# theovincent/iS-DQN

Measured on AMD Instinct MI355X. Metric: gradient-steps/sec (batch=256, K=9, 84x84x4), higher is better.
Workload: dtype bf16x3 (split-bf16 MFMA operands hi+lo, fp32 accumulate)

## Files before the change

is-dqn_amd/csrc/common.h:

```cpp
#pragma once
#include <hip/hip_runtime.h>
#include <stdint.h>
#include <stdio.h>
#include <stdlib.h>

#include "../../include/isdqn_hip.h"

namespace isdqn {

void set_last_error(const char* fmt, ...);

#define ISDQN_HIP_CHECK(expr)                                                                         \
    do {                                                                                              \
        hipError_t _e = (expr);                                                                       \
        if (_e != hipSuccess) {                                                                       \
            ::isdqn::set_last_error("%s failed: %s (%s:%d)", #expr, hipGetErrorString(_e), __FILE__, \
                                    __LINE__);                                                        \
            return ISDQN_ERR_HIP;                                                                     \
        }                                                                                             \
    } while (0)

#define ISDQN_REQUIRE(cond, code, msg)                                         \
    do {                                                                       \
        if (!(cond)) {                                                         \
            ::isdqn::set_last_error("%s (%s:%d)", msg, __FILE__, __LINE__);    \
            return code;                                                       \
        }                                                                      \
    } while (0)

struct FastDiv {
    uint32_t d, m, sh;
    __host__ __device__ FastDiv() : d(1), m(0), sh(0) {}
    __host__ __device__ explicit FastDiv(uint32_t div) : d(div), m(0), sh(0) {
        if (div > 1) {
            uint32_t lg = 0;
            while ((1u << lg) < div) ++lg;
            uint32_t p = 31 + lg;
            m = (uint32_t)(((1ull << p) + div - 1) / div);
            sh = p - 32;
        }
    }
    __host__ __device__ __forceinline__ uint32_t div(uint32_t n) const {
#if defined(__HIP_DEVICE_COMPILE__)
        const uint32_t q = __umulhi(n, m) >> sh;
        return d == 1 ? n : q;
#else
        return d == 1 ? n : (uint32_t)((((uint64_t)n * m) >> 32) >> sh);
#endif
    }
    __host__ __device__ __forceinline__ void divmod(uint32_t n, uint32_t& q, uint32_t& r) const {
        q = div(n);
        r = n - q * d;
    }
};

#if defined(ISDQN_DEV)
#define ISDQN_DEV_ENV(name) (getenv(name) != nullptr)
#else
#define ISDQN_DEV_ENV(name) (false)
#endif

#if defined(ISDQN_DEV)
#define ISDQN_REPORT_OCCUPANCY(kernel, threads, lds_bytes, grid)                                                              \
    do {                                                                                                                      \
        static bool reported_ = false;                                                                                        \
        if (!reported_ && getenv("ISDQN_DEBUG_OCCUPANCY")) {                                                                  \
            reported_ = true;                                                                                                 \
            int nb_ = 0;                                                                                                      \
            if (hipOccupancyMaxActiveBlocksPerMultiprocessor(&nb_, reinterpret_cast<const void*>(kernel), (threads),          \
                                                             (lds_bytes)) == hipSuccess)                                      \
                fprintf(stderr, "[isdqn] %s: grid %d x %d threads, %d B LDS -> %d workgroups per CU\n", __PRETTY_FUNCTION__,  \
                        (int)(grid), (int)(threads), (int)(lds_bytes), nb_);                                                  \
        }                                                                                                                     \
    } while (0)
#else
#define ISDQN_REPORT_OCCUPANCY(kernel, threads, lds_bytes, grid) do {} while (0)
#endif

constexpr int ISDQN_MAX_DEVICES = 16;
static inline int current_device_slot() {
    int d = 0;
    if (hipGetDevice(&d) != hipSuccess || d < 0 || d >= ISDQN_MAX_DEVICES) d = 0;
    return d;
}
struct LdsConfigured {
    int bytes[ISDQN_MAX_DEVICES] = {0};
};
template <class F>
static inline int ensure_dynamic_lds(F kernel, int lds_bytes, LdsConfigured& state) {
    if (lds_bytes <= 65536) return ISDQN_OK;
    const int d = current_device_slot();
    if (lds_bytes > state.bytes[d]) {
        ISDQN_HIP_CHECK(hipFuncSetAttribute(reinterpret_cast<const void*>(kernel), hipFuncAttributeMaxDynamicSharedMemorySize, lds_bytes));
        state.bytes[d] = lds_bytes;
    }
    return ISDQN_OK;
}

static inline int ceil_div(int a, int b) { return (a + b - 1) / b; }
static inline int round_up(int a, int b) { return ceil_div(a, b) * b; }

}

#if defined(ISDQN_EMPTY)
#define ISDQN_EMPTY_KERNEL_RETURN return;
#else
#define ISDQN_EMPTY_KERNEL_RETURN
#endif
```

is-dqn_amd/csrc/conv_img.h:

```cpp
#pragma once
#include "net_problems.h"

namespace isdqn {

__device__ __forceinline__ int column_slot(int c16) { return c16 < 4 ? 8 + c16 : (c16 < 12 ? c16 - 4 : c16); }
struct PixelOrder {
    int strips;
    int n_full;
    int full_w;
    FastDiv d_h8, d_rem, d_w;
    PixelOrder() : strips(0), n_full(0), full_w(0) {}
    PixelOrder(int H, int W, bool use_strips) : strips(use_strips ? 1 : 0), n_full(H * 8 * (W / 8)), full_w(8 * (W / 8)) {
        d_h8 = FastDiv((uint32_t)(H * 8));
        d_rem = FastDiv((uint32_t)(W % 8 ? W % 8 : 1));
        d_w = FastDiv((uint32_t)W);
    }
    __device__ __forceinline__ void map(int n, int& y, int& x) const {
        uint32_t a, b;
        if (!strips) {
            d_w.divmod((uint32_t)n, a, b);
            y = (int)a; x = (int)b;
        } else if (n < n_full) {
            d_h8.divmod((uint32_t)n, a, b);
            y = (int)(b >> 3); x = (int)(a * 8 + (b & 7));
// ... 680 lines not shown
            int pixoff[2], arow[2];
#pragma unroll
            for (int h = 0; h < 2; ++h) {
                int kp = ks * GEMM_BK + tr_row(8 * grp + 4 * h + q);
                arow[h] = kp * p.PA + 4 * pq;
                kp = kp < g.npix ? kp : g.npix - 1;
                uint32_t oy, ox;
                g.d_wout.divmod((uint32_t)kp, oy, ox);
                pixoff[h] = U8 ? ((int)oy * g.stride * p.Wp + (int)ox * g.stride)
                               : ((int)oy * g.stride * p.Wp + (int)ox * g.stride) * p.PPin;
            }
            bf16x8 fa_hi[MT], fa_lo[MT];
#pragma unroll
            for (int mt = 0; mt < MT; ++mt) {
                fa_hi[mt] = tr_frag(dzi + arow[0] + mt * 16, dzi + arow[1] + mt * 16);
                if constexpr (PASSES >= 2)
                    fa_lo[mt] = tr_frag(dzi + p.dz_plane + arow[0] + mt * 16, dzi + p.dz_plane + arow[1] + mt * 16);
            }
#pragma unroll
            for (int t = 0; t < NTW; ++t) {
                const __bf16* b0 = img + pixoff[0] + col_off[t];
                const __bf16* b1 = img + pixoff[1] + col_off[t];
                bf16x8 fb_hi = tr_frag(b0, b1), fb_lo;
                if constexpr (PASSES >= 3) fb_lo = tr_frag(b0 + p.in_plane, b1 + p.in_plane);
#pragma unroll
                for (int mt = 0; mt < MT; ++mt) {
                    if constexpr (PASSES >= 3)
                        mfma_acc(acc[mt][t], fa_hi[mt], fb_lo);
                    if constexpr (PASSES >= 2)
                        mfma_acc(acc[mt][t], fa_lo[mt], fb_hi);
                    mfma_acc(acc[mt][t], fa_hi[mt], fb_hi);
                }
            }
        }
    };
    bool staged = false;
    if constexpr (!U8) {
        if (p.prefetch) {
            staged = true;
            ImagePrefetch<WgradPrefetch<WV>::DZ> ra;
            ImagePrefetch<WgradPrefetch<WV>::IN> rb;
            auto request = [&](int j) {
                request_image_s8<NTHR>(ra, p.dz + (int64_t)j * g.npix * g.cout_p, 1, g.npix, g.cout_p, 0, 0, 1, p.npix_pad, p.PA, tid,
                                       p.d_dzchunk, p.d_npixpad);
                request_image_s8<NTHR>(rb, p.in + (int64_t)j * g.hin * g.win * g.cin_p, g.hin, g.win, g.cin_p, -g.pad, -g.pad, p.R, p.Wp,
                                       p.PPin, tid, p.d_chunk, p.d_Wp);
            };
            request(j0);
            for (int j = j0; j < j1; ++j) {
                __syncthreads();
                commit_image_s8<A_PLANES>(dzi, p.dz_plane, ra);
                commit_image_s8<B_PLANES>(img, p.in_plane, rb);
                __syncthreads();
                if (j == j0) { WG_STAMP(1); } else if (j == j0 + 1) { WG_STAMP(3); }
                if (j + 1 < j1) request(j + 1);
                k_steps();
                if (j == j0) { WG_STAMP(2); } else if (j == j0 + 1) { WG_STAMP(4); }
            }
        }
    }
    if (!staged)
    for (int j = j0; j < j1; ++j) {
        __syncthreads();
        bool dz_done = false;
        if constexpr (U8) {
            if (p.prefetch) {
                ImagePrefetch<WgradPrefetch<WV>::DZ_U8> ra;
                request_image_s8<NTHR>(ra, p.dz + (int64_t)j * g.npix * g.cout_p, 1, g.npix, g.cout_p, 0, 0, 1, p.npix_pad, p.PA, tid,
                                       p.d_dzchunk, p.d_npixpad);
                fill_input_image<U8, PASSES, NTHR>(img, p.in_plane, g, p.fs, p.in, j, -g.pad, p.R, p.Wp, p.PPin, tid, p.d_chunk, p.d_Wp, p.d_R);
                commit_image_s8<A_PLANES>(dzi, p.dz_plane, ra);
                dz_done = true;
            }
        }
        if (!dz_done) {
            fill_image_s8<NTHR, A_PLANES, 8>(dzi, p.dz_plane, p.dz + (int64_t)j * g.npix * g.cout_p, 1, g.npix, g.cout_p, 0, 0, 1, p.npix_pad,
                                             p.PA, tid, p.d_dzchunk, p.d_npixpad);
            fill_input_image<U8, PASSES, NTHR>(img, p.in_plane, g, p.fs, p.in, j, -g.pad, p.R, p.Wp, p.PPin, tid, p.d_chunk, p.d_Wp, p.d_R);
        }
        __syncthreads();
        if (j == j0) { WG_STAMP(1); } else if (j == j0 + 1) { WG_STAMP(3); }
        k_steps();
        if (j == j0) { WG_STAMP(2); } else if (j == j0 + 1) { WG_STAMP(4); }
    }

    float* slab = p.slabs + (int64_t)ig * g.cout_p * g.K;
#pragma unroll
    for (int mt = 0; mt < MT; ++mt)
#pragma unroll
        for (int t = 0; t < NTW; ++t) {
            const int col = cg * p.NC + (wave + WV * t) * 16 + li;
#pragma unroll
            for (int r = 0; r < 4; ++r) {
                const int row = mt * 16 + grp * 4 + r;
#if !defined(ISDQN_NO_STREAMING)
                if (row < g.cout_p && col < g.K) __builtin_nontemporal_store(acc[mt][t][r] * p.scale, (ISDQN_GLOBAL float*)(slab + (int64_t)row * g.K + col));
#else
                if (row < g.cout_p && col < g.K) slab[(int64_t)row * g.K + col] = acc[mt][t][r] * p.scale;
#endif
            }
        }
#if defined(ISDQN_DEV)
    if (p.stamps != nullptr) {
        __builtin_amdgcn_s_waitcnt(0);
        WG_STAMP(5);
    }
#endif
#undef WG_STAMP
}

template <int MT, int NTW, int PASSES, bool U8, int WV = 4>
static int launch_conv_wgrad_img(const ConvWgradImgParams& p, int n_img_groups, hipStream_t st) {
    constexpr int A_PLANES = PASSES >= 2 ? 2 : 1;
    constexpr int B_PLANES = (PASSES >= 3) ? 2 : 1;
    const int lds = (A_PLANES * p.dz_plane + B_PLANES * p.in_plane) * 2;
    static LdsConfigured configured;
    if (int rc = ensure_dynamic_lds(&conv_wgrad_img_kernel<MT, NTW, PASSES, U8, WV>, lds, configured)) return rc;
    ISDQN_REPORT_OCCUPANCY((&conv_wgrad_img_kernel<MT, NTW, PASSES, U8, WV>), 64 * WV, lds, n_img_groups * p.n_col_groups);
    ConvWgradImgParams q = p;
    q.prefetch = 0;
#if !defined(ISDQN_WGRAD_NO_PREFETCH)
    if (!U8 && p.G >= 2 && p.npix_pad * (p.g.cout_p / 8) <= WgradPrefetch<WV>::DZ * 64 * WV &&
        p.R * p.Wp * (p.g.cin_p / 8) <= WgradPrefetch<WV>::IN * 64 * WV)
        q.prefetch = 1;
#if !defined(ISDQN_WGRAD_NO_U8_DZ)
    if (U8 && p.npix_pad * (p.g.cout_p / 8) <= WgradPrefetch<WV>::DZ_U8 * 64 * WV) q.prefetch = 1;
#endif
#endif
    hipLaunchKernelGGL((conv_wgrad_img_kernel<MT, NTW, PASSES, U8, WV>), dim3(n_img_groups * p.n_col_groups),
                       dim3(64 * WV), lds, st, q);
    ISDQN_HIP_CHECK(hipGetLastError());
    return ISDQN_OK;
}


struct ConvDgradImgParams {
    ConvGeom g;
    const float* W;
    const float* dz;
    const float* z_in;
    const float *gamma, *beta;
    int c_in;
    float* dz_in;
    float* part;
    int n_img, T, Kc;
    int Hd, Wd, PPd, bt;
    FastDiv d_chunk, d_Wd, d_T;
    long long* stamps;
    int dz_plane;
    int tiles_per_img;
    int cls_tile_start[5];
    PixelOrder cls_order[4];
    int n_classes;
};

template <int MT, int PASSES, int NT = 2>
__global__ __launch_bounds__(GEMM_THREADS, 2) void conv_dgrad_img_kernel(const ConvDgradImgParams p) {
    ISDQN_EMPTY_KERNEL_RETURN
    constexpr int BM = MT * 16;
    constexpr int A_PLANES = PASSES >= 2 ? 2 : 1;
    constexpr int B_PLANES = PASSES >= 3 ? 2 : 1;
    using GA = TileGeom<BM, true>;
    constexpr int A_STAGE = A_PLANES * GA::ELEMS;
    extern __shared__ __attribute__((aligned(16))) char smem_raw[];
    __bf16* a_stage = reinterpret_cast<__bf16*>(smem_raw);
    __bf16* img = a_stage + 2 * A_STAGE;
    __shared__ float s_part[4][3][64];
    const ConvGeom& g = p.g;
    const int tid = threadIdx.x, lane = tid & 63, wave = tid >> 6, grp = lane >> 4;
#if defined(ISDQN_DEV)
#define ISDQN_STAMP(i)                                                                               \
    if (p.stamps != nullptr && threadIdx.x == 0) {                                                  \
        p.stamps[(int64_t)blockIdx.x * 8 + (i)] = (long long)__builtin_amdgcn_s_memtime();           \
        if ((i) == 0) p.stamps[(int64_t)blockIdx.x * 8 + 7] = (long long)__builtin_amdgcn_s_memrealtime(); \
    }
#define ISDQN_ABLATED(bit) ((p.ablate & (bit)) != 0)
#else
#define ISDQN_STAMP(i)
#define ISDQN_ABLATED(bit) (false)
#endif
    ISDQN_STAMP(0);

    int j, tl;
    xcd_image_tile((int)blockIdx.x, p.n_img, p.tiles_per_img, j, tl);
    int cls = 0;
    while (cls + 1 < p.n_classes && tl >= p.cls_tile_start[cls + 1]) ++cls;
    const int q0 = (tl - p.cls_tile_start[cls]) * (64 * NT);
    const int smask = g.stride - 1;
    const int cy = cls >> g.stride_sh, cx = cls & smask;
    const int Ha = (g.hin - cy + g.stride - 1) >> g.stride_sh, Wb = (g.win - cx + g.stride - 1) >> g.stride_sh;
    const int n_cls_pix = Ha * Wb;
    const int py = (cy + g.pad) & smask, px = (cx + g.pad) & smask;

    __shared__ __attribute__((aligned(16))) float s_gb[2][64];
    float par_v = 0.f;
    {
        const int which = tid >> 6, ch = tid & 63;
        const float* src = which == 0 ? p.gamma : p.beta;
        const bool ok = tid < 128 && ch < g.cin_p && p.gamma != nullptr;
        ISDQN_BOUNDS_CHECK(ok ? src + ch : zero_chunk(), 4, 13);
        par_v = *(const ISDQN_GLOBAL float*)(ok ? src + ch : zero_chunk());
    }

    const int nsteps = (p.Kc + GEMM_BK - 1) / GEMM_BK;
    const int k_last = p.Kc - 8;
    constexpr int A_PER = GA::PER_THREAD;
    int a_ci0[A_PER], a_kk[A_PER], a_lds[A_PER];
    bool a_on[A_PER];
#pragma unroll
    for (int i = 0; i < A_PER; ++i) {
        int c = tid + i * GEMM_THREADS;
        a_on[i] = c < GA::CHUNKS;
        if (!a_on[i]) c = 0;
        const int kk = c / (BM / 8), rc = c % (BM / 8);
        a_ci0[i] = rc * 8; a_kk[i] = kk;
        a_lds[i] = tr_row(kk) * GA::PITCH + rc * 8;
    }
    constexpr int PF = 4;
    float sa[PF][A_PER][8];
    auto fetch = [&](int slot, int k0) {
#pragma unroll
        for (int i = 0; i < A_PER; ++i) {
            const int k = k0 + a_kk[i];
            const bool ok = (k < p.Kc) && (a_ci0[i] < g.cin_p);
            uint32_t jt, co;
            g.d_coutp.divmod(ok ? (uint32_t)k : 0u, jt, co);
            uint32_t jy_u, jx_u;
            p.d_T.divmod(jt, jy_u, jx_u);
            const int jy = (int)jy_u, jx = (int)jx_u;
            const int ky = py + g.stride * jy, kx = px + g.stride * jx;
            load8_aligned(ok ? p.W + ((int64_t)co * g.K + (ky * g.ksz + kx) * g.cin_p + a_ci0[i]) : zero_chunk(), sa[slot][i]);
        }
    };
    auto stash = [&](int slot, int stage) {
        __bf16* a_hi = a_stage + stage * A_STAGE;
        __bf16* a_lo = a_hi + GA::ELEMS;
#pragma unroll
        for (int i = 0; i < A_PER; ++i) {
            if (GA::CHUNKS % GEMM_THREADS != 0 && !a_on[i]) continue;
            bf16x8 hi, lo;
            if constexpr (PASSES >= 2) {
                s8_unpack(sa[slot][i], hi, lo);
                *reinterpret_cast<bf16x8*>(a_lo + a_lds[i]) = lo;
            } else {
                s8_unpack_hi(sa[slot][i], hi);
            }
            *reinterpret_cast<bf16x8*>(a_hi + a_lds[i]) = hi;
        }
    };

    const int nsteps_p = (nsteps + PF - 1) / PF * PF;
    const int rot = (int)((blockIdx.x >> 3) % (unsigned)nsteps);
    auto slice = [&](int s) {
        const int k = s + rot;
        return s < nsteps ? (k >= nsteps ? k - nsteps : k) : nsteps_p;
    };
#pragma unroll
    for (int d = 0; d < PF; ++d) fetch(d, slice(d) * GEMM_BK);

    fill_image_s8<GEMM_THREADS, B_PLANES, 8>(img, p.dz_plane, p.dz + (int64_t)j * g.hout * g.wout * g.cout_p, g.hout, g.wout, g.cout_p,
                                             -p.bt, -p.bt, p.Hd, p.Wd, p.PPd, tid, p.d_chunk, p.d_Wd);

    ISDQN_STAMP(1);
    int b_org[NT], pix_iy[NT], pix_ix[NT];
    bool pix_ok[NT];
#pragma unroll
    for (int nt = 0; nt < NT; ++nt) {
        int q = q0 + wave * (16 * NT) + nt * 16 + column_slot(lane & 15);
        pix_ok[nt] = q < n_cls_pix;
        q = pix_ok[nt] ? q : n_cls_pix - 1;
        int a, b;
        p.cls_order[cls].map(q, a, b);
        const int iy = cy + g.stride * a, ix = cx + g.stride * b;
        pix_iy[nt] = iy; pix_ix[nt] = ix;
        const int oyb = (iy + g.pad - py) >> g.stride_sh, oxb = (ix + g.pad - px) >> g.stride_sh;
        b_org[nt] = ((oyb + p.bt) * p.Wd + oxb + p.bt) * p.PPd;
    }

    f32x4 acc[MT][NT];
#pragma unroll
    for (int mt = 0; mt < MT; ++mt)
#pragma unroll
        for (int nt = 0; nt < NT; ++nt) mfma_init(acc[mt][nt]);

    struct Frags {
        bf16x8 a_hi[MT], a_lo[MT], b_hi[NT], b_lo[NT];
    };
    auto read_frags = [&](int stage, int kk, Frags& f) {
        const __bf16* a_hi = a_stage + stage * A_STAGE;
        const __bf16* a_lo = a_hi + GA::ELEMS;
#pragma unroll
        for (int mt = 0; mt < MT; ++mt) {
            f.a_hi[mt] = read_frag<true, GA::PITCH>(a_hi, mt * 16, lane);
            if constexpr (PASSES >= 2) f.a_lo[mt] = read_frag<true, GA::PITCH>(a_lo, mt * 16, lane);
        }
        int kq = kk * GEMM_BK + grp * 8;
        kq = kq < k_last ? kq : k_last;
        uint32_t jt, co;
        g.d_coutp.divmod((uint32_t)kq, jt, co);
        uint32_t jy_u, jx_u;
        p.d_T.divmod(jt, jy_u, jx_u);
        const int jy = (int)jy_u, jx = (int)jx_u;
        const int tap_off = -(jy * p.Wd + jx) * p.PPd + (int)co;
#pragma unroll
        for (int nt = 0; nt < NT; ++nt) {
            const __bf16* src = img + b_org[nt] + tap_off;
            f.b_hi[nt] = *reinterpret_cast<const bf16x8*>(src);
            if constexpr (PASSES >= 3) f.b_lo[nt] = *reinterpret_cast<const bf16x8*>(src + p.dz_plane);
        }
    };
    auto mfma_step = [&](const Frags& f) {
#pragma unroll
        for (int nt = 0; nt < NT; ++nt)
#pragma unroll
            for (int mt = 0; mt < MT; ++mt) {
                if constexpr (PASSES >= 3)
                    mfma_acc(acc[mt][nt], f.a_hi[mt], f.b_lo[nt]);
                if constexpr (PASSES >= 2)
                    mfma_acc(acc[mt][nt], f.a_lo[mt], f.b_hi[nt]);
                mfma_acc(acc[mt][nt], f.a_hi[mt], f.b_hi[nt]);
            }
    };

    float zpre[NT][MT][4];
#pragma unroll
    for (int nt = 0; nt < NT; ++nt) {
        const int64_t pixel = ((int64_t)j * g.hin + pix_iy[nt]) * g.win + pix_ix[nt];
#pragma unroll
        for (int mt = 0; mt < MT; ++mt) {
            const int ch0 = mt * 16 + grp * 4;
            ISDQN_BOUNDS_CHECK(ch0 < g.cin_p ? p.z_in + pixel * g.cin_p + ch0 : zero_chunk(), 16, 12);
            const ISDQN_GLOBAL f32x4* zp = (const ISDQN_GLOBAL f32x4*)(ch0 < g.cin_p ? p.z_in + pixel * g.cin_p + ch0 : zero_chunk());
            const f32x4 zq = *zp;
            zpre[nt][mt][0] = zq[0]; zpre[nt][mt][1] = zq[1]; zpre[nt][mt][2] = zq[2]; zpre[nt][mt][3] = zq[3];
        }
    }

    static_assert(PF % 2 == 0 && PF >= 4, "the fragment sets alternate with the step parity; steps 0..3 are pre-fetched");
    Frags fr[2];
    if (tid < 128) s_gb[tid >> 6][tid & 63] = par_v;
    stash(0, 0);
    stash(1, 1);
    fetch(0, slice(PF) * GEMM_BK);
    fetch(1, slice(PF + 1) * GEMM_BK);
    __syncthreads();
    ISDQN_STAMP(2);
    read_frags(0, slice(0), fr[0]);
    __syncthreads();
    constexpr bool INTERLEAVED = PASSES == 3 && MT == 4 && A_PER == 1 && GA::CHUNKS == GEMM_THREADS;
    auto tap_offset_of = [&](int kk) {
        int kq = kk * GEMM_BK + grp * 8;
        kq = kq < k_last ? kq : k_last;
        uint32_t jt, co, jy_u, jx_u;
        g.d_coutp.divmod((uint32_t)kq, jt, co);
        p.d_T.divmod(jt, jy_u, jx_u);
        return -((int)jy_u * p.Wd + (int)jx_u) * p.PPd + (int)co;
    };
    int tap_next = INTERLEAVED ? tap_offset_of(slice(1)) : 0;
    for (int s0 = 0; s0 < nsteps_p; s0 += PF) {
#pragma unroll
        for (int u = 0; u < PF; ++u) {
            const int s = s0 + u;
            if constexpr (INTERLEAVED) {
                const Frags& fc = fr[u & 1];
                Frags& fn = fr[(u + 1) & 1];
                const __bf16* na_hi = a_stage + ((s + 1) & 1) * A_STAGE;
                const __bf16* na_lo = na_hi + GA::ELEMS;
                const int tap_off = tap_next;
                const int slot = (u + 2) % PF;
                __bf16* st_hi = a_stage + (s & 1) * A_STAGE + a_lds[0];
                __bf16* st_lo = st_hi + GA::ELEMS;
                bf16x8 c_hi, c_lo;
                constexpr int NM = 12 * NT;
                __builtin_amdgcn_sched_barrier(0);
#pragma unroll
                for (int jm = 0; jm < NM; ++jm) {
                    const int pass = jm / (4 * NT), nt = (jm >> 2) % NT, mt = jm & 3;
                    mfma_acc(acc[mt][nt], pass == 1 ? fc.a_lo[mt] : fc.a_hi[mt], pass == 0 ? fc.b_lo[nt] : fc.b_hi[nt]);
                    if (jm < 4) fn.a_hi[jm] = read_frag<true, GA::PITCH>(na_hi, jm * 16, lane);
                    else if (jm < 8) fn.a_lo[jm - 4] = read_frag<true, GA::PITCH>(na_lo, (jm - 4) * 16, lane);
                    else if (jm < 8 + NT) fn.b_hi[jm - 8] = *reinterpret_cast<const bf16x8*>(img + b_org[jm - 8] + tap_off);
                    else if (jm < 8 + 2 * NT) fn.b_lo[jm - 8 - NT] = *reinterpret_cast<const bf16x8*>(img + b_org[jm - 8 - NT] + tap_off + p.dz_plane);
                    else if constexpr (NT == 2) {
                        if (jm == 12) s8_unpack(sa[slot][0], c_hi, c_lo);
                        else if (jm == 16) *reinterpret_cast<bf16x8*>(st_lo) = c_lo;
                        else if (jm == 17) *reinterpret_cast<bf16x8*>(st_hi) = c_hi;
                        else if (jm == 18) fetch(slot, slice(s + 2 + PF) * GEMM_BK);
                        else if (jm == 19) tap_next = tap_offset_of(slice(s + 2));
                    } else {
                        if (jm == 10) {
                            s8_unpack(sa[slot][0], c_hi, c_lo);
                            *reinterpret_cast<bf16x8*>(st_lo) = c_lo;
                            *reinterpret_cast<bf16x8*>(st_hi) = c_hi;
                        } else if (jm == 11) {
                            fetch(slot, slice(s + 2 + PF) * GEMM_BK);
                            tap_next = tap_offset_of(slice(s + 2));
                        }
                    }
                    __builtin_amdgcn_sched_barrier(0);
                }
                __syncthreads();
                continue;
            }
            read_frags((s + 1) & 1, slice(s + 1), fr[(u + 1) & 1]);
            mfma_step(fr[u & 1]);
            stash((u + 2) % PF, s & 1);
            fetch((u + 2) % PF, slice(s + 2 + PF) * GEMM_BK);
            constexpr int N_MFMA = MT * NT * (PASSES >= 3 ? 3 : PASSES);
#pragma unroll
            for (int i = 0; i < N_MFMA; ++i) {
                __builtin_amdgcn_sched_group_barrier(0x008, 1, 0);
                if (i < N_MFMA / 2) __builtin_amdgcn_sched_group_barrier(0x100, 1, 0);
                __builtin_amdgcn_sched_group_barrier(0x002, 2, 0);
            }
            __syncthreads();
        }
    }

    ISDQN_STAMP(3);
    float ga[MT][4], be[MT][4];
#pragma unroll
    for (int mt = 0; mt < MT; ++mt) {
        const int ch0 = (mt * 16 + grp * 4) & 63;
        const float4 g4 = *reinterpret_cast<const float4*>(&s_gb[0][ch0]);
        const float4 e4 = *reinterpret_cast<const float4*>(&s_gb[1][ch0]);
        ga[mt][0] = g4.x; ga[mt][1] = g4.y; ga[mt][2] = g4.z; ga[mt][3] = g4.w;
        be[mt][0] = e4.x; be[mt][1] = e4.y; be[mt][2] = e4.z; be[mt][3] = e4.w;
    }
    float dg[MT][4], db[MT][4], dbias[MT][4];
#pragma unroll
    for (int mt = 0; mt < MT; ++mt)
#pragma unroll
        for (int r = 0; r < 4; ++r) dg[mt][r] = db[mt][r] = dbias[mt][r] = 0.f;
    const float inv_c = 1.f / (float)p.c_in;
#pragma unroll
    for (int nt = 0; nt < NT; ++nt) {
        const int64_t pixel = ((int64_t)j * g.hin + pix_iy[nt]) * g.win + pix_ix[nt];
        float zv[MT][4];
#pragma unroll
        for (int mt = 0; mt < MT; ++mt)
#pragma unroll
            for (int r = 0; r < 4; ++r) zv[mt][r] = zpre[nt][mt][r];
        float out[MT][4];
        if (p.gamma != nullptr) {
            float s1 = 0.f, s2 = 0.f;
#pragma unroll
            for (int mt = 0; mt < MT; ++mt)
#pragma unroll
                for (int r = 0; r < 4; ++r) {
                    const bool ok = (mt * 16 + grp * 4 + r) < p.c_in;
                    s1 += ok ? zv[mt][r] : 0.f;
                    s2 += ok ? zv[mt][r] * zv[mt][r] : 0.f;
                }
            s1 += __shfl_xor(s1, 16); s1 += __shfl_xor(s1, 32);
            s2 += __shfl_xor(s2, 16); s2 += __shfl_xor(s2, 32);
            const float mean = s1 * inv_c;
            const float rstd = rsqrtf(fmaxf(s2 * inv_c - mean * mean, 0.f) + 1e-6f);
            float xh[MT][4], gg[MT][4], m1 = 0.f, m2 = 0.f;
#pragma unroll
            for (int mt = 0; mt < MT; ++mt)
#pragma unroll
                for (int r = 0; r < 4; ++r) {
                    const bool ok = pix_ok[nt] && (mt * 16 + grp * 4 + r) < p.c_in;
                    xh[mt][r] = (zv[mt][r] - mean) * rstd;
                    const float y = xh[mt][r] * ga[mt][r] + be[mt][r];
                    const float dy = (ok && y > 0.f) ? acc[mt][nt][r] : 0.f;
                    dg[mt][r] += dy * xh[mt][r];
                    db[mt][r] += dy;
                    gg[mt][r] = dy * ga[mt][r];
                    m1 += gg[mt][r];
                    m2 += gg[mt][r] * xh[mt][r];
                }
            m1 += __shfl_xor(m1, 16); m1 += __shfl_xor(m1, 32);
            m2 += __shfl_xor(m2, 16); m2 += __shfl_xor(m2, 32);
            m1 *= inv_c;
            m2 *= inv_c;
#pragma unroll
            for (int mt = 0; mt < MT; ++mt)
#pragma unroll
                for (int r = 0; r < 4; ++r) {
                    const bool ok = pix_ok[nt] && (mt * 16 + grp * 4 + r) < p.c_in;
                    out[mt][r] = ok ? rstd * (gg[mt][r] - m1 - xh[mt][r] * m2) : 0.f;
                    dbias[mt][r] += out[mt][r];
                }
        } else {
#pragma unroll
            for (int mt = 0; mt < MT; ++mt)
#pragma unroll
                for (int r = 0; r < 4; ++r) {
                    const bool ok = pix_ok[nt] && (mt * 16 + grp * 4 + r) < p.c_in;
                    out[mt][r] = (ok && zv[mt][r] > 0.f) ? acc[mt][nt][r] : 0.f;
                    dbias[mt][r] += out[mt][r];
                }
        }
        if (pix_ok[nt]) {
#pragma unroll
            for (int mt = 0; mt < MT; ++mt) {
                const int ch0 = mt * 16 + grp * 4;
                if (ch0 < g.cin_p)
                    s8_store_quad_paired(p.dz_in + pixel * g.cin_p, ch0, out[mt][0], out[mt][1], out[mt][2], out[mt][3]);
            }
        }
    }
#pragma unroll
    for (int mt = 0; mt < MT; ++mt)
#pragma unroll
        for (int r = 0; r < 4; ++r) {
            dg[mt][r] = row16_sum(dg[mt][r]);
            db[mt][r] = row16_sum(db[mt][r]);
            dbias[mt][r] = row16_sum(dbias[mt][r]);
            if ((lane & 15) == 0) {
                const int ch = mt * 16 + grp * 4 + r;
                s_part[wave][0][ch] = dg[mt][r];
                s_part[wave][1][ch] = db[mt][r];
                s_part[wave][2][ch] = dbias[mt][r];
            }
        }
    __syncthreads();
    for (int i = tid; i < 3 * g.cin_p; i += GEMM_THREADS) {
        const int which = (i >= g.cin_p) + (i >= 2 * g.cin_p), c = i - which * g.cin_p;
        p.part[((int64_t)blockIdx.x * 3 + which) * g.cin_p + c] =
            s_part[0][which][c] + s_part[1][which][c] + s_part[2][which][c] + s_part[3][which][c];
    }
    ISDQN_STAMP(4);
#if defined(ISDQN_DEV)
    if (p.stamps != nullptr) {
        __builtin_amdgcn_s_waitcnt(0);
        ISDQN_STAMP(5);
    }
#endif
#undef ISDQN_STAMP
#undef ISDQN_ABLATED
}

constexpr int REDUCE_MAX_JOBS = 4;
struct ReduceJobs {
    const float* part[REDUCE_MAX_JOBS];
    float* out[REDUCE_MAX_JOBS];
    int n_rows[REDUCE_MAX_JOBS], width[REDUCE_MAX_JOBS];
    int block_start[REDUCE_MAX_JOBS + 1];
    int n;
};
__global__ __launch_bounds__(256) void reduce_rows_kernel(const ReduceJobs jobs) {
    ISDQN_EMPTY_KERNEL_RETURN
    __shared__ float s_red[32][8];
    int job = 0;
#pragma unroll
    for (int i = 1; i < REDUCE_MAX_JOBS; ++i)
        if (i < jobs.n && (int)blockIdx.x >= jobs.block_start[i]) job = i;
    const float* __restrict__ part = jobs.part[job];
    float* __restrict__ out = jobs.out[job];
    const int n_rows = jobs.n_rows[job], width = jobs.width[job];
    const int col = ((int)blockIdx.x - jobs.block_start[job]) * 8 + (threadIdx.x & 7), rl = threadIdx.x >> 3;
    float s = 0.f;
    if (col < width) {
        int r = rl;
        for (; r + 7 * 32 < n_rows; r += 8 * 32) {
            float v[8];
#pragma unroll
            for (int u = 0; u < 8; ++u) v[u] = part[(int64_t)(r + u * 32) * width + col];
#pragma unroll
            for (int u = 0; u < 8; ++u) s += v[u];
        }
        for (; r < n_rows; r += 32) s += part[(int64_t)r * width + col];
    }
    s_red[rl][threadIdx.x & 7] = s;
    __syncthreads();
    if (rl == 0 && col < width) {
        float t = 0.f;
#pragma unroll
        for (int k = 0; k < 32; ++k) t += s_red[k][threadIdx.x & 7];
        out[col] = t;
    }
}

template <int MT, int PASSES, int NT = 2>
static int launch_conv_dgrad_img(const ConvDgradImgParams& p, hipStream_t st) {
    constexpr int A_PLANES = PASSES >= 2 ? 2 : 1;
    constexpr int B_PLANES = PASSES >= 3 ? 2 : 1;
    using GA = TileGeom<MT * 16, true>;
    const int lds = (2 * A_PLANES * GA::ELEMS + B_PLANES * p.dz_plane) * 2;
    static LdsConfigured configured;
    if (int rc = ensure_dynamic_lds(&conv_dgrad_img_kernel<MT, PASSES, NT>, lds, configured)) return rc;
    ISDQN_REPORT_OCCUPANCY((&conv_dgrad_img_kernel<MT, PASSES, NT>), GEMM_THREADS, lds, p.n_img * p.tiles_per_img);
    hipLaunchKernelGGL((conv_dgrad_img_kernel<MT, PASSES, NT>), dim3(p.n_img * p.tiles_per_img), dim3(GEMM_THREADS), lds, st, p);
    ISDQN_HIP_CHECK(hipGetLastError());
    return ISDQN_OK;
}

}
```

is-dqn_amd/csrc/net_launch.h:

```cpp
#pragma once
#if defined(ISDQN_DEV)
static long long* g_stamps = nullptr;
static int g_stamp_layer = -1;
static char g_stamp_name[32] = "";
extern "C" int isdqn_debug_set_stamps(void* buf, const char* layer_name) {
    g_stamps = (long long*)buf;
    g_stamp_layer = buf ? 0 : -1;
    snprintf(g_stamp_name, sizeof(g_stamp_name), "%s", layer_name ? layer_name : "");
    return ISDQN_OK;
}
static long long* stamps_for(const char* kernel_tag) {
    return (g_stamp_layer >= 0 && strcmp(kernel_tag, g_stamp_name) == 0) ? g_stamps : nullptr;
}
#else
static long long* stamps_for(const char*) { return nullptr; }
#endif

__global__ __launch_bounds__(256) void split_params_kernel(const float* __restrict__ p, float* __restrict__ mirror, int64_t n_groups) {
    const int64_t g = (int64_t)blockIdx.x * 256 + threadIdx.x;
    if (g >= n_groups) return;
    float v[8];
    load8_aligned(p + g * 8, v);
    s8_store_group(mirror + g * 8, v);
}
// ... 303 lines not shown
        int cy = c / l.stride, cx = c % l.stride;
        int Ha = (l.hin - cy + l.stride - 1) / l.stride, Wb = (l.win - cx + l.stride - 1) / l.stride;
        p.tile_start[c] = acc;
        p.cls_d_hw[c] = FastDiv((uint32_t)(Ha * Wb));
        p.cls_d_w[c] = FastDiv((uint32_t)Wb);
        acc += ceil_div(n_img * Ha * Wb, 128);
    }
    p.tile_start[p.n_classes] = acc;
    return launch_gemm(p, acc, st);
}

template <int PASSES, bool U8>
static int launch_conv_wgrad(const Layer& l, const NetInput& in, const float* act_in, const float* dz, float* slabs,
                             int n_img, hipStream_t st) {
    ConvWgrad<PASSES, U8> p;
    p.g = conv_geom(l);
    p.n_pix = n_img * l.npix;
    p.DZ = MatSrc{dz, l.cout_p, p.n_pix, l.cout_p, 1};
    p.in = act_in;
    p.fs = FrameSrc{in.frames, in.frame_stride, in.frame_ids, l.cin, in.paired_B, l.hin, l.win, in.id_pitch, in.id_off};
    p.slabs = slabs;
    p.scale = U8 ? (1.0f / 255.0f) : 1.0f;
    p.tiles_n = ceil_div(l.K, 64);
    int ksteps = ceil_div(p.n_pix, GEMM_BK);
    p.steps_per_split = ceil_div(ksteps, l.gw_slabs);
    p.splits = ceil_div(ksteps, p.steps_per_split);
    return launch_gemm(p, p.tiles_n * p.splits, st);
}
static int conv_wgrad_img(const Layer& l, bool x3, const NetInput& in, const float* act_in, const float* dz, float* slabs,
                          int n_img, hipStream_t st, int* slabs_out) {
    *slabs_out = 0;
    if (!l.wgi_ntw || n_img != 0 && ceil_div(n_img, l.wgi_G) > l.gw_slabs) return ISDQN_OK;
    ConvWgradImgParams wp;
    wp.g = conv_geom(l);
    const int passes = x3 ? (l.is_u8 ? 2 : 3) : 1;
    const int mt = l.cout_p <= 32 ? 2 : 4;
    int lds_unused_R, Wp, plane;
    conv_img_geometry(wp.g, l.is_u8, l.cin, 1, mt, 1, lds_unused_R, Wp, plane);
    wp.R = l.stride * (l.hout - 1) + l.ksz;
    wp.Wp = Wp;
    wp.PPin = l.cin_p;
    for (int pad = 0; pad <= 24; pad += 8)
        if ((l.stride * (l.cin_p + pad)) % 32 == 16) { wp.PPin = l.cin_p + pad; break; }
    wp.in_plane = l.is_u8 ? l.cin * wp.R * Wp : wp.R * Wp * wp.PPin;
    wp.PA = l.cout_p + (l.cout_p % 32 == 0 ? 16 : 8);
    wp.npix_pad = round_up(l.npix, 32);
    wp.dz_plane = wp.npix_pad * wp.PA;
    const int lds = ((passes >= 2 ? 2 : 1) * wp.dz_plane + (passes >= 3 ? 2 : 1) * wp.in_plane) * 2;
    if (lds > 150 * 1024 || (l.is_u8 && (l.win < 8 || l.cin > 4))) return ISDQN_OK;
    wp.d_chunk = FastDiv((uint32_t)(l.is_u8 ? Wp / 8 : l.cin_p / 8));
    wp.d_Wp = FastDiv((uint32_t)Wp);
    wp.d_R = FastDiv((uint32_t)wp.R);
    wp.d_dzchunk = FastDiv((uint32_t)(l.cout_p / 8));
    wp.d_npixpad = FastDiv((uint32_t)wp.npix_pad);
    wp.dz = dz; wp.in = act_in;
    wp.fs = FrameSrc{in.frames, in.frame_stride, in.frame_ids, l.cin, in.paired_B, l.hin, l.win, in.id_pitch, in.id_off};
    wp.slabs = slabs;
    wp.scale = l.is_u8 ? (1.0f / 255.0f) : 1.0f;
    wp.n_img = n_img; wp.G = l.wgi_G;
    wp.NC = 64 * l.wgi_ntw;
    wp.n_col_groups = l.K / wp.NC;
    wp.d_ncg = FastDiv((uint32_t)wp.n_col_groups);
    {
        char tag[32];
        snprintf(tag, sizeof(tag), "wgrad:%s", l.name);
        wp.stamps = stamps_for(tag);
    }
    const int groups = ceil_div(n_img, l.wgi_G);
    *slabs_out = groups;
#define WGI(MT_, NTW_, P_, U_) return launch_conv_wgrad_img<MT_, NTW_, P_, U_>(wp, groups, st)
#define WGI8(MT_, NTW_, P_, U_) return launch_conv_wgrad_img<MT_, NTW_, P_, U_, 8>(wp, groups, st)
    if (l.is_u8) {
        if (mt == 2) { if (l.wgi_ntw == 4) { if (passes == 2) WGI(2, 4, 2, true); else WGI(2, 4, 1, true); }
                       if (l.wgi_ntw == 2) { if (passes == 2) WGI(2, 2, 2, true); else WGI(2, 2, 1, true); } }
        else         { if (l.wgi_ntw == 4) { if (passes == 2) WGI(4, 4, 2, true); else WGI(4, 4, 1, true); }
                       if (l.wgi_ntw == 2) { if (passes == 2) WGI(4, 2, 2, true); else WGI(4, 2, 1, true); } }
    } else {
        if (mt == 2) { if (l.wgi_ntw == 4) { if (passes == 3) WGI(2, 4, 3, false); else WGI(2, 4, 1, false); }
                       if (l.wgi_ntw == 3) { if (passes == 3) WGI(2, 3, 3, false); else WGI(2, 3, 1, false); }
                       if (l.wgi_ntw == 2) { if (passes == 3) WGI(2, 2, 3, false); else WGI(2, 2, 1, false); } }
        else         {
                       static const bool w4 = ISDQN_DEV_ENV("ISDQN_WGRAD_4WAVES");
                       if (l.wgi_ntw == 8 && !w4) { if (passes == 3) WGI8(4, 4, 3, false); else WGI8(4, 4, 1, false); }
                       if (l.wgi_ntw == 9) { if (passes == 3) WGI(4, 9, 3, false); else WGI(4, 9, 1, false); }
                       if (l.wgi_ntw == 8) { if (passes == 3) WGI(4, 8, 3, false); else WGI(4, 8, 1, false); }
                       if (l.wgi_ntw == 4) { if (passes == 3) WGI(4, 4, 3, false); else WGI(4, 4, 1, false); }
                       if (l.wgi_ntw == 3) { if (passes == 3) WGI(4, 3, 3, false); else WGI(4, 3, 1, false); }
                       if (l.wgi_ntw == 2) { if (passes == 3) WGI(4, 2, 3, false); else WGI(4, 2, 1, false); } }
    }
#undef WGI
#undef WGI8
    *slabs_out = 0;
    return ISDQN_OK;
}

static void add_reduce_job(ReduceJobs& jobs, const float* part, int n_rows, int width, float* out) {
    const int i = jobs.n++;
    jobs.part[i] = part; jobs.out[i] = out; jobs.n_rows[i] = n_rows; jobs.width[i] = width;
    jobs.block_start[i + 1] = jobs.block_start[i] + ceil_div(width, 8);
}

static int conv_dgrad_img(const Layer& l, const Layer& below, bool x3, const float* params, const float* wmir, const float* dz, float* ws,
                          int n_img, hipStream_t st, bool* done, ReduceJobs* jobs) {
    *done = false;
    if (!l.dgi_tiles || below.part_rows < n_img * l.dgi_tiles) return ISDQN_OK;
    ConvDgradImgParams dp;
    dp.g = conv_geom(l);
    dp.W = wmir + l.w_off;
    dp.dz = dz;
    dp.z_in = ws + below.z_off;
    dp.gamma = below.has_ln ? params + below.g_off : nullptr;
    dp.beta = below.has_ln ? params + below.be_off : nullptr;
    dp.c_in = below.out_f;
    dp.dz_in = ws + below.dz_off;
    dp.part = ws + below.part_off;
    dp.n_img = n_img;
    dp.T = l.ksz / l.stride;
    dp.Kc = dp.T * dp.T * l.cout_p;
#if defined(ISDQN_DGRAD_WIDE_BORDER)
    dp.bt = dp.T - 1;
#else
    dp.bt = dp.T - 1 - l.pad / l.stride > 0 ? dp.T - 1 - l.pad / l.stride : 0;
#endif
    const int need_h = (l.hin - 1 + l.pad) / l.stride + 1, need_w = (l.win - 1 + l.pad) / l.stride + 1;
    dp.Hd = dp.bt + (l.hout > need_h ? l.hout : need_h);
    dp.Wd = dp.bt + (l.wout > need_w ? l.wout : need_w);
    dp.PPd = l.cout_p + ((16 - l.cout_p % 32) + 32) % 32;
    dp.dz_plane = dp.Hd * dp.Wd * dp.PPd;
    dp.d_chunk = FastDiv((uint32_t)(l.cout_p / 8));
    dp.d_Wd = FastDiv((uint32_t)dp.Wd);
    dp.d_T = FastDiv((uint32_t)dp.T);
    {
        char tag[32];
        snprintf(tag, sizeof(tag), "dgrad:%s", l.name);
        dp.stamps = stamps_for(tag);
    }
    dp.n_classes = l.stride * l.stride;
    int acc = 0;
    for (int c = 0; c < dp.n_classes; ++c) {
        int cy = c / l.stride, cx = c % l.stride;
        int Ha = (l.hin - cy + l.stride - 1) / l.stride, Wb = (l.win - cx + l.stride - 1) / l.stride;
        dp.cls_tile_start[c] = acc;
        dp.cls_order[c] = PixelOrder(Ha, Wb, Ha * Wb <= 128);
        acc += ceil_div(Ha * Wb, l.dgi_tile_pix);
    }
    dp.cls_tile_start[dp.n_classes] = acc;
    dp.tiles_per_img = acc;
    const int mt = l.cin_p <= 32 ? 2 : 4;
    const int passes = x3 ? 3 : 1;
    const int lds = (2 * (passes >= 2 ? 2 : 1) * 32 * (mt * 16 + 16) + (passes >= 3 ? 2 : 1) * dp.dz_plane) * 2;
    if (lds > 150 * 1024) return ISDQN_OK;
    int rc;
    ISDQN_REQUIRE(acc == l.dgi_tiles, ISDQN_ERR_ARG, "data-gradient tiling differs from the plan's");
#if ISDQN_DGRAD_TILE64_BELOW > 0
    if (l.dgi_tile_pix == 64) {
        if (passes == 3) rc = mt == 2 ? launch_conv_dgrad_img<2, 3, 1>(dp, st) : launch_conv_dgrad_img<4, 3, 1>(dp, st);
        else rc = mt == 2 ? launch_conv_dgrad_img<2, 1, 1>(dp, st) : launch_conv_dgrad_img<4, 1, 1>(dp, st);
    } else
#endif
    if (passes == 3) rc = mt == 2 ? launch_conv_dgrad_img<2, 3>(dp, st) : launch_conv_dgrad_img<4, 3>(dp, st);
    else rc = mt == 2 ? launch_conv_dgrad_img<2, 1>(dp, st) : launch_conv_dgrad_img<4, 1>(dp, st);
    if (rc) return rc;
    add_reduce_job(*jobs, ws + below.part_off, n_img * dp.tiles_per_img, 3 * below.out_p, ws + below.red_off);
    *done = true;
    return ISDQN_OK;
}

static int conv_wgrad_slabs(const Layer& l, int n_img) {
    int ksteps = ceil_div(n_img * l.npix, GEMM_BK);
    int sps = ceil_div(ksteps, l.gw_slabs);
    return ceil_div(ksteps, sps);
}

static inline const BnSite* bn_site_of(const Plan& P, int layer);
static int bn_site_forward(const BnSite& b, const float* params, float* ws, int rows, bool running, hipStream_t st);
static int bn_site_backward(const BnSite& b, const float* params, float* ws, float* dy, int rows, bool apply, hipStream_t st);
struct HeadSel {
    int on0 = 0, tg0 = 0, K = 0;
};

enum class LearnMode { Loss, Learn, GradOnly };
struct LearnCall {
    const isdqn_net_config* cfg = nullptr;
    LearnMode mode = LearnMode::Loss;
    float *params = nullptr, *adam_m = nullptr, *adam_v = nullptr;
    int32_t* adam_count = nullptr;
    const float* target_params = nullptr;
    const isdqn_batch* batch = nullptr;
    float *losses = nullptr, *loss_accum = nullptr, *q_values = nullptr, *targets = nullptr;
    double* priorities = nullptr;
    float* grad_out = nullptr;
    float* ws = nullptr;
    hipStream_t st = nullptr;
    HeadSel sel;
    float weight_decay = 0.f;
    int32_t decay_kinds = 0;
    float wd(int kind) const { return ((decay_kinds >> kind) & 1) ? weight_decay : 0.f; }
    float cql_alpha = 0.f;
    bool mixture = false;
    const float* mix_alpha = nullptr;
    int32_t n_mix = 0;
    bool learn() const { return mode != LearnMode::Loss; }
    bool update() const { return mode == LearnMode::Learn; }
};

static int resolve_heads(const Plan& P, HeadSel& sel) {
    if (sel.K <= 0) return sel = HeadSel{P.oh, 0, P.K}, ISDQN_OK;
    ISDQN_REQUIRE(sel.on0 >= 0 && sel.tg0 >= 0 && sel.on0 + sel.K <= P.n_heads && sel.tg0 + sel.K <= P.n_heads && sel.K <= P.K, ISDQN_ERR_ARG,
                  "head selection outside the network's heads");
    return ISDQN_OK;
}

static void moments_of_a_gradient_only_pass(LearnCall& call) { call.adam_m = call.adam_v = call.params; }


struct AdamList {
    std::vector<AdamEntry> e;
    AdamList() { e.reserve(ADAM_MAX_ENTRIES); }
    void add(int64_t p_off, int64_t size, const float* g, int n_slabs, int64_t stride, float wd) {
        e.push_back(AdamEntry{p_off, size, stride, g, n_slabs, 0, wd});
    }
    AdamTable table(size_t e0, int per_block = 64) const {
        AdamTable tab;
        tab.n = 0;
        tab.total_blocks = 0;
        for (size_t k = e0; k < e.size() && k < e0 + ADAM_MAX_ENTRIES; ++k) {
            AdamEntry& t = tab.e[tab.n++];
            t = e[k];
            t.block_start = tab.total_blocks;
            tab.total_blocks += (int)((t.size + per_block - 1) / per_block);
        }
        return tab;
    }
    int launch(hipStream_t st, const Plan& P, const isdqn_net_config* cfg, float* params, float* adam_m, float* adam_v, float* ws, float* grad_out,
               bool update) const {
        for (size_t e0 = 0; e0 < e.size(); e0 += ADAM_MAX_ENTRIES) {
            const AdamTable tab = table(e0);
            hipLaunchKernelGGL(adam_kernel, dim3(tab.total_blocks), dim3(256), 0, st, tab, params, adam_m, adam_v, ws + P.adam_tab_off, cfg->learning_rate,
                               cfg->adam_b1, cfg->adam_b2, cfg->adam_eps, grad_out, ws + P.wsplit_off, update ? 1 : 0);
            ISDQN_HIP_CHECK(hipGetLastError());
        }
        return ISDQN_OK;
    }
};
static int adam_launch(const AdamList& list, hipStream_t st, const Plan& P, const LearnCall& c) {
    return list.launch(st, P, c.cfg, c.params, c.adam_m, c.adam_v, c.ws, c.grad_out, c.update());
}

static int loss_finalize(const Plan& P, const isdqn_net_config* cfg, float* ws, int n_blk, int K, int width, float* losses, float* loss_accum,
                         bool head_bias_grad, int32_t* adam_count, hipStream_t st) {
    float* loss_part = ws + P.lpart_off;
    hipLaunchKernelGGL(loss_finalize_kernel, dim3(ceil_div(K, 16) + ceil_div(width, 16)), dim3(256), 0, st, loss_part, loss_part + (int64_t)n_blk * K, n_blk,
                       P.B, K, width, losses, loss_accum, head_bias_grad ? ws + P.dbh_off : nullptr, adam_count, cfg->adam_b1, cfg->adam_b2,
                       ws + P.adam_tab_off);
    ISDQN_HIP_CHECK(hipGetLastError());
    return ISDQN_OK;
}

static inline const float* batch_discount(const isdqn_batch* batch) {
    return (batch->flags & ISDQN_BATCH_DISCOUNT) ? reinterpret_cast<const isdqn_batch_discount*>(batch)->discount : nullptr;
}
static inline void batch_decay(const isdqn_batch* batch, float* weight_decay, int32_t* decay_kinds) {
    const bool has = batch != nullptr && (batch->flags & ISDQN_BATCH_WEIGHT_DECAY);
    const isdqn_batch_decay* d = reinterpret_cast<const isdqn_batch_decay*>(batch);
    *weight_decay = has ? d->weight_decay : 0.f;
    *decay_kinds = has ? d->decay_kinds : 0;
}
static inline float batch_conservative(const isdqn_batch* batch) {
    const bool has = batch != nullptr && (batch->flags & ISDQN_BATCH_CONSERVATIVE);
    return has ? reinterpret_cast<const isdqn_batch_conservative*>(batch)->cql_alpha : 0.f;
}
static inline bool batch_mixture(const isdqn_batch* batch, const float** alpha, int32_t* n_mix) {
    const bool has = batch != nullptr && (batch->flags & ISDQN_BATCH_MIXTURE);
    const isdqn_batch_mixture* m = reinterpret_cast<const isdqn_batch_mixture*>(batch);
    *alpha = has ? m->alpha : nullptr;
    *n_mix = has ? m->n_mix : 0;
    return has;
}
static int check_conservative(float cql_alpha) {
    ISDQN_REQUIRE(cql_alpha >= 0.f && cql_alpha <= 3.4028234e38f, ISDQN_ERR_ARG, "cql_alpha must be finite and >= 0");
    return ISDQN_OK;
}
static int check_decay(float weight_decay, int32_t decay_kinds) {
    ISDQN_REQUIRE(weight_decay >= 0.f && weight_decay <= 3.4028234e38f, ISDQN_ERR_ARG, "weight_decay must be finite and >= 0");
    ISDQN_REQUIRE((decay_kinds & ~ISDQN_DECAY_KINDS_ALL) == 0, ISDQN_ERR_ARG, "decay_kinds: bits 0..6 only (kinds 7 and 8 are running statistics)");
    ISDQN_REQUIRE(weight_decay == 0.f || decay_kinds != 0, ISDQN_ERR_ARG, "weight_decay > 0 needs at least one kind in decay_kinds");
    return ISDQN_OK;
}

static int loss_and_finalize(const Plan& P, const LearnCall& c, bool double_q = false, const float* val_rows = nullptr,
                             const float* state_val_rows = nullptr) {
    const isdqn_net_config* cfg = c.cfg;
    const isdqn_batch* batch = c.batch;
    float* ws = c.ws;
    const int B = P.B, K = c.sel.K, on0 = c.sel.on0, tg0 = c.sel.tg0;
    const bool learn = c.learn();
    const Munchausen mu{cfg->munchausen_tau, cfg->munchausen_alpha, cfg->munchausen_clip};
    if (state_val_rows == nullptr) state_val_rows = ws + P.out_off;
    const float* mun_rows = mu.tau > 0.f ? state_val_rows : nullptr;
    const float* next_rows = ws + P.out_off + (int64_t)B * P.nlog_p;
    if (val_rows == nullptr) val_rows = next_rows;
    const float* sel_rows = double_q ? next_rows : nullptr;
    const int R = P.head_nb > 0 ? rows_per_wg(K, P.head_nb) : 0;
    const int n_blk = R ? ceil_div(B, R) : ceil_div(B, TD_ROWS);
    float* loss_part = ws + P.lpart_off;
    HeadLossArgs a{};
// ... 116 lines not shown
```

Baseline: 4348.

## Process multiple dgrad tiles per workgroup, reusing the staged image and prefetching the next tile

Measured after the change: 4255. -2.1%, worse.

```diff
diff --git a/is-dqn_amd/csrc/common.h b/is-dqn_amd/csrc/common.h
--- a/is-dqn_amd/csrc/common.h
+++ b/is-dqn_amd/csrc/common.h
@@ -56,8 +56,10 @@
 
 #if defined(ISDQN_DEV)
 #define ISDQN_DEV_ENV(name) (getenv(name) != nullptr)
+#define ISDQN_DEV_ENV_INT(name) (getenv(name) != nullptr ? atoi(getenv(name)) : 0)
 #else
 #define ISDQN_DEV_ENV(name) (false)
+#define ISDQN_DEV_ENV_INT(name) (0)
 #endif
 
 #if defined(ISDQN_DEV)
@@ -83,6 +85,16 @@
     if (hipGetDevice(&d) != hipSuccess || d < 0 || d >= ISDQN_MAX_DEVICES) d = 0;
     return d;
 }
+static inline int device_cu_count() {
+    static int cus[ISDQN_MAX_DEVICES] = {0};
+    const int d = current_device_slot();
+    if (cus[d] == 0) {
+        int n = 0;
+        if (hipDeviceGetAttribute(&n, hipDeviceAttributeMultiprocessorCount, d) != hipSuccess || n <= 0) n = 256;
+        cus[d] = n;
+    }
+    return cus[d];
+}
 struct LdsConfigured {
     int bytes[ISDQN_MAX_DEVICES] = {0};
 };
diff --git a/is-dqn_amd/csrc/conv_img.h b/is-dqn_amd/csrc/conv_img.h
--- a/is-dqn_amd/csrc/conv_img.h
+++ b/is-dqn_amd/csrc/conv_img.h
@@ -856,6 +856,7 @@
     int cls_tile_start[5];
     PixelOrder cls_order[4];
     int n_classes;
+    int cpw;
 };
 
 template <int MT, int PASSES, int NT = 2>
@@ -875,26 +876,39 @@
 #if defined(ISDQN_DEV)
 #define ISDQN_STAMP(i)                                                                               \
     if (p.stamps != nullptr && threadIdx.x == 0) {                                                  \
-        p.stamps[(int64_t)blockIdx.x * 8 + (i)] = (long long)__builtin_amdgcn_s_memtime();           \
-        if ((i) == 0) p.stamps[(int64_t)blockIdx.x * 8 + 7] = (long long)__builtin_amdgcn_s_memrealtime(); \
+        p.stamps[(int64_t)wg_tile * 8 + (i)] = (long long)__builtin_amdgcn_s_memtime();              \
+        if ((i) == 0) {                                                                             \
+            p.stamps[(int64_t)wg_tile * 8 + 7] = (long long)__builtin_amdgcn_s_memrealtime();        \
+            p.stamps[(int64_t)wg_tile * 8 + 6] = (long long)pass;                                    \
+        }                                                                                           \
     }
 #define ISDQN_ABLATED(bit) ((p.ablate & (bit)) != 0)
 #else
 #define ISDQN_STAMP(i)
 #define ISDQN_ABLATED(bit) (false)
 #endif
+
+    int j, tgrp;
+    xcd_image_tile((int)blockIdx.x, p.n_img, p.tiles_per_img / p.cpw, j, tgrp);
+    const int tl0 = tgrp * p.cpw;
+    const int smask = g.stride - 1;
+    const int nsteps = (p.Kc + GEMM_BK - 1) / GEMM_BK;
+    int q0, cy, cx, n_cls_pix, py, px, rot, cls, wg_of;
+    auto set_tile = [&](int tl) {
+        cls = 0;
+        while (cls + 1 < p.n_classes && tl >= p.cls_tile_start[cls + 1]) ++cls;
+        q0 = (tl - p.cls_tile_start[cls]) * (64 * NT);
+        cy = cls >> g.stride_sh; cx = cls & smask;
+        const int Ha = (g.hin - cy + g.stride - 1) >> g.stride_sh, Wb = (g.win - cx + g.stride - 1) >> g.stride_sh;
+        n_cls_pix = Ha * Wb;
+        py = (cy + g.pad) & smask; px = (cx + g.pad) & smask;
+        const int T = p.tiles_per_img;
+        wg_of = (T > 1 && j < (p.n_img / 8) * 8) ? (j >> 3) * 8 * T + tl * 8 + (j & 7) : j * T + tl;
+        rot = (int)((unsigned)(wg_of >> 3) % (unsigned)nsteps);
+    };
+    set_tile(tl0);
+    int pass = 0, wg_tile = wg_of;
     ISDQN_STAMP(0);
-
-    int j, tl;
-    xcd_image_tile((int)blockIdx.x, p.n_img, p.tiles_per_img, j, tl);
-    int cls = 0;
-    while (cls + 1 < p.n_classes && tl >= p.cls_tile_start[cls + 1]) ++cls;
-    const int q0 = (tl - p.cls_tile_start[cls]) * (64 * NT);
-    const int smask = g.stride - 1;
-    const int cy = cls >> g.stride_sh, cx = cls & smask;
-    const int Ha = (g.hin - cy + g.stride - 1) >> g.stride_sh, Wb = (g.win - cx + g.stride - 1) >> g.stride_sh;
-    const int n_cls_pix = Ha * Wb;
-    const int py = (cy + g.pad) & smask, px = (cx + g.pad) & smask;
 
     __shared__ __attribute__((aligned(16))) float s_gb[2][64];
     float par_v = 0.f;
@@ -906,7 +920,6 @@
         par_v = *(const ISDQN_GLOBAL float*)(ok ? src + ch : zero_chunk());
     }
 
-    const int nsteps = (p.Kc + GEMM_BK - 1) / GEMM_BK;
     const int k_last = p.Kc - 8;
     constexpr int A_PER = GA::PER_THREAD;
     int a_ci0[A_PER], a_kk[A_PER], a_lds[A_PER];
@@ -954,7 +967,6 @@
     };
 
     const int nsteps_p = (nsteps + PF - 1) / PF * PF;
-    const int rot = (int)((blockIdx.x >> 3) % (unsigned)nsteps);
     auto slice = [&](int s) {
         const int k = s + rot;
         return s < nsteps ? (k >= nsteps ? k - nsteps : k) : nsteps_p;
@@ -964,8 +976,10 @@
 
     fill_image_s8<GEMM_THREADS, B_PLANES, 8>(img, p.dz_plane, p.dz + (int64_t)j * g.hout * g.wout * g.cout_p, g.hout, g.wout, g.cout_p,
                                              -p.bt, -p.bt, p.Hd, p.Wd, p.PPd, tid, p.d_chunk, p.d_Wd);
+    if (tid < 128) s_gb[tid >> 6][tid & 63] = par_v;
 
     ISDQN_STAMP(1);
+    for (;;) {
     int b_org[NT], pix_iy[NT], pix_ix[NT];
     bool pix_ok[NT];
 #pragma unroll
@@ -1042,7 +1056,6 @@
 
     static_assert(PF % 2 == 0 && PF >= 4, "the fragment sets alternate with the step parity; steps 0..3 are pre-fetched");
     Frags fr[2];
-    if (tid < 128) s_gb[tid >> 6][tid & 63] = par_v;
     stash(0, 0);
     stash(1, 1);
     fetch(0, slice(PF) * GEMM_BK);
@@ -1122,6 +1135,10 @@
     }
 
     ISDQN_STAMP(3);
+    const bool more = pass + 1 < p.cpw;
+    if (more) set_tile(tl0 + pass + 1);
+#pragma unroll
+    for (int d = 0; d < PF; ++d) fetch(d, (more ? slice(d) : nsteps_p) * GEMM_BK);
     float ga[MT][4], be[MT][4];
 #pragma unroll
     for (int mt = 0; mt < MT; ++mt) {
@@ -1223,7 +1240,7 @@
     __syncthreads();
     for (int i = tid; i < 3 * g.cin_p; i += GEMM_THREADS) {
         const int which = (i >= g.cin_p) + (i >= 2 * g.cin_p), c = i - which * g.cin_p;
-        p.part[((int64_t)blockIdx.x * 3 + which) * g.cin_p + c] =
+        p.part[((int64_t)wg_tile * 3 + which) * g.cin_p + c] =
             s_part[0][which][c] + s_part[1][which][c] + s_part[2][which][c] + s_part[3][which][c];
     }
     ISDQN_STAMP(4);
@@ -1233,6 +1250,13 @@
         ISDQN_STAMP(5);
     }
 #endif
+    if (!more) break;
+    ++pass;
+    wg_tile = wg_of;
+    __syncthreads();
+    ISDQN_STAMP(0);
+    ISDQN_STAMP(1);
+    }
 #undef ISDQN_STAMP
 #undef ISDQN_ABLATED
 }
@@ -1284,10 +1308,13 @@
     constexpr int B_PLANES = PASSES >= 3 ? 2 : 1;
     using GA = TileGeom<MT * 16, true>;
     const int lds = (2 * A_PLANES * GA::ELEMS + B_PLANES * p.dz_plane) * 2;
+    ISDQN_REQUIRE((p.cpw == 1 || p.cpw == 2 || p.cpw == 4) && p.tiles_per_img % p.cpw == 0, ISDQN_ERR_ARG,
+                  "data gradient: tiles per workgroup must be 1, 2 or 4 and divide the tiles of an image");
+    const int grid = p.n_img * (p.tiles_per_img / p.cpw);
     static LdsConfigured configured;
     if (int rc = ensure_dynamic_lds(&conv_dgrad_img_kernel<MT, PASSES, NT>, lds, configured)) return rc;
-    ISDQN_REPORT_OCCUPANCY((&conv_dgrad_img_kernel<MT, PASSES, NT>), GEMM_THREADS, lds, p.n_img * p.tiles_per_img);
-    hipLaunchKernelGGL((conv_dgrad_img_kernel<MT, PASSES, NT>), dim3(p.n_img * p.tiles_per_img), dim3(GEMM_THREADS), lds, st, p);
+    ISDQN_REPORT_OCCUPANCY((&conv_dgrad_img_kernel<MT, PASSES, NT>), GEMM_THREADS, lds, grid);
+    hipLaunchKernelGGL((conv_dgrad_img_kernel<MT, PASSES, NT>), dim3(grid), dim3(GEMM_THREADS), lds, st, p);
     ISDQN_HIP_CHECK(hipGetLastError());
     return ISDQN_OK;
 }
diff --git a/is-dqn_amd/csrc/net_launch.h b/is-dqn_amd/csrc/net_launch.h
--- a/is-dqn_amd/csrc/net_launch.h
+++ b/is-dqn_amd/csrc/net_launch.h
@@ -479,6 +479,13 @@
     if (lds > 150 * 1024) return ISDQN_OK;
     int rc;
     ISDQN_REQUIRE(acc == l.dgi_tiles, ISDQN_ERR_ARG, "data-gradient tiling differs from the plan's");
+    dp.cpw = (l.dgi_tile_pix == 128 && acc % 2 == 0 && n_img * acc > 2 * device_cu_count()) ? 2 : 1;
+#if defined(ISDQN_DEV)
+    if (const int forced = ISDQN_DEV_ENV_INT("ISDQN_DGRAD_CPW")) {
+        const char* only = getenv("ISDQN_DGRAD_CPW_LAYER");
+        if (only == nullptr || strcmp(only, l.name) == 0) dp.cpw = forced;
+    }
+#endif
 #if ISDQN_DGRAD_TILE64_BELOW > 0
     if (l.dgi_tile_pix == 64) {
         if (passes == 3) rc = mt == 2 ? launch_conv_dgrad_img<2, 3, 1>(dp, st) : launch_conv_dgrad_img<4, 3, 1>(dp, st);
```
